# smdesai/mlx-swift-audio

Measured on AMD Instinct MI355X. Metric: audio-sec/s (Whisper large-v3-turbo b=32) at 1/2/4/8 GPU; codec samples/s, higher is better.
Workload: dtype bf16; 1 GPU; Whisper large-v3-turbo bf16, batch=32x30 s synthetic clips per MI355X, log-mel+encode+greedy decode (T=0, timestamps, max_tokens 448, one window per clip), random-init N(0,0.02^2) weights; clips_per_gpu=32, global_batch=32, parallelism=dp1, replicas=3, exchange=none, schedule=pipelined

## Files before the change

include/mia.h:

```cpp
#ifndef MIA_H
#define MIA_H

#include <stddef.h>
#include <stdint.h>

#ifdef __cplusplus
extern "C" {
#endif

typedef struct mia_ctx mia_ctx;
typedef struct mia_whisper mia_whisper;
typedef struct mia_codec mia_codec;
typedef struct mia_lm mia_lm;
typedef struct mia_s3tok mia_s3tok;

typedef enum {
  MIA_OK = 0,
  MIA_ERR_INVALID_ARGUMENT = -1,
  MIA_ERR_MODEL_NOT_LOADED = -2,
  MIA_ERR_INVALID_AUDIO = -3,
  MIA_ERR_OUT_OF_MEMORY = -4,
  MIA_ERR_DEVICE = -5,
  MIA_ERR_UNSUPPORTED = -6
} mia_status;
// ... 18 lines not shown
                       int64_t pad_right, int64_t n_frames_out, void* mel, int out_dtype, int mem);

int mia_logmel_s3(mia_ctx* ctx, const float* pcm, const int64_t* offs, int B, int n_mels,
                  int64_t pad_right, int64_t n_frames_out, void* mel, int out_dtype, int mem);

int64_t mia_mel_s3gen_frames(int64_t n_samples);
int mia_mel_s3gen(mia_ctx* ctx, const float* pcm, int64_t n_samples, float* mel, int mem);

int64_t mia_resample_linear_len(int64_t n_samples, float scale);
int mia_resample_linear(mia_ctx* ctx, const float* x, int64_t n_samples, float scale, float* out, int mem);
int64_t mia_resample_sinc_len(int64_t n_samples, int from_rate, int to_rate);
int mia_resample_sinc_table(int from_rate, int to_rate, float* table, int capacity, int* L_out, int* taps_out);
int mia_resample_sinc(mia_ctx* ctx, const float* x, int64_t n_samples, int from_rate, int to_rate, float* out, int64_t out_capacity,
                      int64_t* n_out, int mem);

int mia_dp_shard_range(int n_items, int rank, int world, int* lo, int* hi);
int mia_dp_shard_cap(int n_items, int world);
int mia_dp_unpack_host(const int32_t* gathered, int n_items, int world, int L, int32_t* dense);
int mia_dp_available(void);
int mia_dp_unique_id(mia_ctx* ctx, void* id128);
int mia_dp_init(mia_ctx* ctx, int rank, int world, const void* unique_id);
int mia_dp_shutdown(mia_ctx* ctx);
int mia_dp_gather_tokens(mia_ctx* ctx, const int32_t* local_tokens, const int32_t* local_counts, int b_local, int L, int n_items,
                         int32_t* all_tokens, int32_t* all_counts);

int mia_op_linear(mia_ctx* ctx, const void* x, int64_t lda, const void* w, const float* bias, const float* r, int64_t ldr,
                  void* y, int64_t ldy, int M, int N, int K, int act, int dtype, int out_f32, int variant, int mem);

int mia_op_linear_epi(mia_ctx* ctx, const void* x, int64_t lda, const void* w, const float* bias, void* y, int64_t ldy, void* vt, int M, int N,
                      int K, int epi, int T, int H, int Tpad, int batch, int dtype, int out_f32, int variant, int mem);

int mia_op_attention_h64(mia_ctx* ctx, const void* qk, int64_t ld_qk, const void* vt, void* out, int64_t ld_out, int B, int T, int H, int Tpad,
                         int dtype, int mem);

int mia_op_conv1d_f32(mia_ctx* ctx, const float* x, int64_t ldx, int T_in, const float* w, const float* bias, const float* r, float* y,
                      int64_t ldy, int T_out, int N, int Cin, int taps, int stride, int dil, int pad, int act);

int mia_dequant_affine(mia_ctx* ctx, const uint32_t* wq, const void* scales, const void* biases, int64_t rows, int64_t cols,
                       int group_size, int bits, int scale_dtype, void* out, int out_dtype, int mem);

int mia_op_attention_f32(mia_ctx* ctx, const float* q, int64_t ldq, const float* k, int64_t ldk, const float* v, int64_t ldv, float* out,
                         int64_t ldo, int B, int T, int H, float scale);

typedef struct {
  const float* X; int64_t ldx; int32_t T_in;
  const float* W; int64_t ldw; int64_t w_phase_stride;
  const float* bias;
  const float* alpha; const float* ralpha;
  float lrelu_slope;
  float* Y; int64_t ldy; int32_t T_out;
  int32_t y_row_mul, y_row_off, y_phase_step;
  const float* R; const float* R2; int64_t ldr;
  const float* noise;
  float out_scale;
  int32_t M, N, Cin, taps, dil, pad;
  int32_t x_row_mul;
  int32_t act;
  int32_t tanh_out;
  const int32_t* phase_len; int32_t x_phase_step;
  int32_t n_seq; int64_t x_seq_step, y_seq_step;
  const int32_t* seq_len; const int32_t* noise_seq_off;
} mia_conv_gemm_desc;
int mia_op_conv_gemm_f32(mia_ctx* ctx, const mia_conv_gemm_desc* d, int phases);

int mia_op_attention_f32_ex(mia_ctx* ctx, const float* q, int64_t ldq, const float* k, int64_t ldk, const float* v, int64_t ldv, const float* p,
                            int64_t ldp, const float* bias_u, const float* bias_v, float* out, int64_t ldo, int B, int T, int H, float scale,
// ... 256 lines not shown
```

mlx-swift-audio_amd/csrc/attention.hip:

```cpp
#include <type_traits>

#include "mia_device.h"
#include "ops.h"

namespace {

constexpr int KV_TILE = 64;
constexpr int TILE_BYTES = 64 * 128;

__device__ __forceinline__ int swap23(int r) {
  return (r & ~12) | ((r & 4) << 1) | ((r & 8) >> 1);
}

template <typename T>
__global__ __launch_bounds__(256, 2) void enc_attention_kernel(const uint16_t* __restrict__ qk, int64_t ld_qk,
                                                               const uint16_t* __restrict__ vt, uint16_t* __restrict__ out,
                                                               int64_t ld_out, int T_len, int Tpad, int H, float scale_log2) {
  __shared__ __attribute__((aligned(16))) char lds[4 * TILE_BYTES];
  const int tid = threadIdx.x, lane = tid & 63, wave = tid >> 6;
  const int nqb = (T_len + 127) / 128;
  int lin = blockIdx.x;
  {
    const int nwg = gridDim.x, q = nwg / 8, r = nwg % 8, xcd = lin % 8;
    lin = (xcd < r ? xcd * (q + 1) : r * (q + 1) + (xcd - r) * q) + lin / 8;
  }
  const int qb = lin % nqb, hb = lin / nqb;
  const int h = hb % H, b = hb / H;
  const int D = H * 64;
  const int q0 = qb * 128 + wave * 32;
  const int lq = lane & 31, lh = lane >> 5;

  s16x8 qf[4];
  {
    int q = q0 + lq; q = q < T_len ? q : T_len - 1;
    const uint16_t* qp = qk + ((int64_t)b * T_len + q) * ld_qk + h * 64 + 8 * lh;
#pragma unroll
    for (int ks = 0; ks < 4; ++ks) qf[ks] = *reinterpret_cast<const s16x8*>(qp + 16 * ks);
  }

  const int s_row = tid >> 3, s_chk = tid & 7;
  const uint16_t* kbase = qk + (int64_t)b * T_len * ld_qk + D + h * 64 + s_chk * 8;
  const uint16_t* vbase = vt + ((int64_t)b * H + h) * 64 * Tpad + s_chk * 8;
  int s_dst[2];
#pragma unroll
  for (int i = 0; i < 2; ++i) {
    const int row = s_row + 32 * i;
    s_dst[i] = row * 128 + ((s_chk ^ ((row >> 1) & 7)) << 4);
  }
  u32x4 rk[2], rv[2];
  auto load_regs = [&](int key0) {
#pragma unroll
    for (int i = 0; i < 2; ++i) {
      const int row = s_row + 32 * i;
      int key = key0 + row; key = key < T_len ? key : T_len - 1;
      rk[i] = *reinterpret_cast<const u32x4*>(kbase + (int64_t)key * ld_qk);
      rv[i] = *reinterpret_cast<const u32x4*>(vbase + (int64_t)row * Tpad + key0);
    }
  };
  auto write_lds = [&](int buf) {
    char* base = lds + buf * 2 * TILE_BYTES;
#pragma unroll
    for (int i = 0; i < 2; ++i) {
      *reinterpret_cast<u32x4*>(base + s_dst[i]) = rk[i];
      *reinterpret_cast<u32x4*>(base + TILE_BYTES + s_dst[i]) = rv[i];
    }
  };

  f32x16 acc_o[2];
#pragma unroll
  for (int i = 0; i < 2; ++i)
#pragma unroll
    for (int r = 0; r < 16; ++r) acc_o[i][r] = 0.f;
  float m_run = -INFINITY, l_run = 0.f;

  const int krow = swap23(lq);
  const int ntiles = (T_len + KV_TILE - 1) / KV_TILE;
  auto tile = [&](int kt, int cur, auto tail_tag) {
    constexpr bool TAIL = decltype(tail_tag)::value;
    const int key0 = kt * KV_TILE;
    if (kt + 1 < ntiles) load_regs(key0 + KV_TILE);
    const char* sk = lds + cur * 2 * TILE_BYTES;
    const char* sv = sk + TILE_BYTES;

    f32x16 acc_s[2];
#pragma unroll
    for (int kb = 0; kb < 2; ++kb) {
#pragma unroll
      for (int r = 0; r < 16; ++r) acc_s[kb][r] = 0.f;
      const int row = kb * 32 + krow;
#pragma unroll
      for (int ks = 0; ks < 4; ++ks) {
        const s16x8 kf = *reinterpret_cast<const s16x8*>(sk + row * 128 + (((2 * ks + lh) ^ ((row >> 1) & 7)) << 4));
        acc_s[kb] = T::mfma32(kf, qf[ks], acc_s[kb]);
      }
    }
    float mloc = -INFINITY;
#pragma unroll
    for (int kb = 0; kb < 2; ++kb)
#pragma unroll
      for (int r = 0; r < 16; ++r) {
        if (TAIL) {
          const int i = (r & 3) + 8 * (r >> 2) + 4 * lh;
          if (key0 + kb * 32 + swap23(i) >= T_len) acc_s[kb][r] = -INFINITY;
        }
        mloc = fmaxf(mloc, acc_s[kb][r]);
      }
    mloc = fmaxf(mloc, __shfl_xor(mloc, 32, 64));
    constexpr float LAZY_LOG2 = 8.0f;
    const bool grow = (mloc - m_run) * scale_log2 > LAZY_LOG2;
    if (__builtin_amdgcn_ballot_w64(grow) != 0ull) {
      const float m_new = grow ? mloc : m_run;
      const float alpha = __builtin_amdgcn_exp2f((m_run - m_new) * scale_log2);
      m_run = m_new;
      l_run *= alpha;
#pragma unroll
      for (int db = 0; db < 2; ++db)
#pragma unroll
        for (int r = 0; r < 16; ++r) acc_o[db][r] *= alpha;
    }
    const float neg_mc = -m_run * scale_log2;
    float lsum = 0.f;
    s16x8 pf[2][2];
#pragma unroll
    for (int kb = 0; kb < 2; ++kb) {
      float p[16];
#pragma unroll
      for (int r = 0; r < 16; ++r) {
        p[r] = __builtin_amdgcn_exp2f(fmaf(acc_s[kb][r], scale_log2, neg_mc));
        lsum += p[r];
      }
#pragma unroll
      for (int s = 0; s < 2; ++s) {
        u32x4 w;
#pragma unroll
        for (int j = 0; j < 4; ++j) w[j] = pack2<T>(p[8 * s + 2 * j], p[8 * s + 2 * j + 1]);
        pf[kb][s] = __builtin_bit_cast(s16x8, w);
      }
    }
    l_run += lsum;

#pragma unroll
    for (int db = 0; db < 2; ++db) {
      const int row = db * 32 + lq;
#pragma unroll
      for (int kb = 0; kb < 2; ++kb)
#pragma unroll
        for (int s = 0; s < 2; ++s) {
          const int chk = kb * 4 + 2 * s + lh;
          const s16x8 vf = *reinterpret_cast<const s16x8*>(sv + row * 128 + ((chk ^ ((row >> 1) & 7)) << 4));
          acc_o[db] = T::mfma32(vf, pf[kb][s], acc_o[db]);
        }
    }
    if (kt + 1 < ntiles) write_lds(cur ^ 1);
    __syncthreads();
  };
  load_regs(0);
  write_lds(0);
  __syncthreads();
  const int nfull = T_len / KV_TILE;
  int cur = 0;
  for (int kt = 0; kt < nfull; ++kt) { tile(kt, cur, std::false_type{}); cur ^= 1; }
  if (nfull < ntiles) tile(nfull, cur, std::true_type{});

  l_run += __shfl_xor(l_run, 32, 64);
  const float inv = 1.0f / l_run;
  const int q = q0 + lq;
  if (q < T_len) {
    uint16_t* op = out + ((int64_t)b * T_len + q) * ld_out + h * 64 + 4 * lh;
#pragma unroll
    for (int db = 0; db < 2; ++db)
#pragma unroll
      for (int g = 0; g < 4; ++g) {
        const float o0 = acc_o[db][4 * g + 0] * inv, o1 = acc_o[db][4 * g + 1] * inv;
        const float o2 = acc_o[db][4 * g + 2] * inv, o3 = acc_o[db][4 * g + 3] * inv;
        *reinterpret_cast<u32x2*>(op + db * 32 + 8 * g) = (u32x2){pack2<T>(o0, o1), pack2<T>(o2, o3)};
      }
  }
}

}

const char* mia_enc_attention_check(int B, int T, int H, int Tpad, int64_t ld_qk, int64_t ld_out) {
  if (B <= 0 || T <= 0 || H <= 0) return "attention: B, T, H must be > 0";
  if (Tpad % 64 || Tpad < T) return "attention: Tpad must be a multiple of 64 and >= T";
  if (ld_qk % 8 || ld_out % 4) return "attention: row strides must keep 16-byte (qk) / 8-byte (out) alignment";
  return nullptr;
}

int mia_enc_attention_launch(const void* qk, int64_t ld_qk, const void* vt, void* out, int64_t ld_out, int B, int T, int H,
                             int Tpad, int dtype, hipStream_t s) {
  dim3 grid(((T + 127) / 128) * H * B), block(256);
  const float scale_log2 = 0.125f * 1.4426950408889634f;
  if (dtype == MIA_F16)
    hipLaunchKernelGGL((enc_attention_kernel<F16>), grid, block, 0, s, (const uint16_t*)qk, ld_qk, (const uint16_t*)vt,
                       (uint16_t*)out, ld_out, T, Tpad, H, scale_log2);
  else
    hipLaunchKernelGGL((enc_attention_kernel<BF16>), grid, block, 0, s, (const uint16_t*)qk, ld_qk, (const uint16_t*)vt,
                       (uint16_t*)out, ld_out, T, Tpad, H, scale_log2);
  return hipGetLastError() == hipSuccess ? 0 : -1;
}
```

mlx-swift-audio_amd/csrc/ops.h:

```cpp
#pragma once
#include <hip/hip_runtime.h>
#include <stdint.h>

#include "../../include/mia.h"

const char* mia_norm_check(int M, int D, int64_t ldx, int64_t ldy);
int mia_norm_launch(const float* x, int64_t ldx, const float* gamma, const float* beta, void* y, int64_t ldy, int M, int D,
                    float eps, bool rms, int out_dtype, hipStream_t s);

const char* mia_enc_attention_check(int B, int T, int H, int Tpad, int64_t ld_qk, int64_t ld_out);
int mia_enc_attention_launch(const void* qk, int64_t ld_qk, const void* vt, void* out, int64_t ld_out, int B, int T, int H,
                             int Tpad, int dtype, hipStream_t s);

struct AttnF32Args {
  const float* q = nullptr; int64_t ldq = 0;
  const float* k = nullptr; int64_t ldk = 0;
  const float* v = nullptr; int64_t ldv = 0;
  const float* p = nullptr; int64_t ldp = 0;
  const float* bias_u = nullptr; const float* bias_v = nullptr;
  float* out = nullptr; int64_t ldo = 0;
  int B = 1, T = 0, H = 0;
  float scale = 0.125f;
  const int32_t* seq_len = nullptr;
  int chunk = 0;
};
const char* mia_attn_f32_check(const AttnF32Args& a);
int mia_attn_f32_launch(const AttnF32Args& a, hipStream_t s);

struct Attn128Args {
  const void* q = nullptr; int64_t ldq = 0;
  const void* k = nullptr; int64_t ldk = 0;
  const void* v = nullptr; int64_t ldv = 0;
  void* out = nullptr; int64_t ldo = 0;
  int B = 1, T = 0, H = 0;
  float scale = 0.08838834764831845f;
  const int32_t* seq_len = nullptr;
  int dtype = MIA_BF16;
};
const char* mia_attn128_check(const Attn128Args& a);
int mia_attn128_launch(const Attn128Args& a, hipStream_t s);

struct FsmnArgs {
  float* x = nullptr; int64_t ldx = 0;
  const void* v = nullptr; int64_t ldv = 0;
  const float* w = nullptr;
// ... 7 lines not shown
```

mlx-swift-audio_amd/csrc/ops_abi.hip:

```cpp
#include "gemm.h"
#include "mia_internal.h"
#include "ops.h"

extern "C" int mia_op_linear(mia_ctx* ctx, const void* x, int64_t lda, const void* w, const float* bias, const float* r, int64_t ldr,
                             void* y, int64_t ldy, int M, int N, int K, int act, int dtype, int out_f32, int variant, int mem) {
  if (!ctx) return MIA_ERR_INVALID_ARGUMENT;
  MIA_CHECK_ARG(ctx, x && w && y, "op_linear: null pointer");
  MIA_CHECK_ARG(ctx, dtype == MIA_BF16 || dtype == MIA_F16, "op_linear: dtype must be MIA_BF16 or MIA_F16");
  MIA_CHECK_ARG(ctx, mem == MIA_MEM_HOST || mem == MIA_MEM_DEVICE, "op_linear: bad mem");
  MIA_CHECK_ARG(ctx, M > 0 && N > 0 && K > 0 && lda >= K && ldy >= N && (!r || ldr >= N), "op_linear: bad shape");
  MIA_HIP(ctx, hipSetDevice(ctx->device));
  GemmArgs g;
  g.M = M; g.N = N; g.K = K; g.lda = lda; g.ldc = ldy; g.ldr = ldr; g.act = act; g.out_f32 = out_f32 ? 1 : 0; g.variant = variant;
  const size_t xb = (size_t)M * lda * 2, wb = (size_t)N * K * 2, yb = (size_t)M * ldy * (out_f32 ? 4 : 2);
  const size_t bb = bias ? (size_t)N * 4 : 0, rb = r ? (size_t)M * ldr * 4 : 0;
  if (mem == MIA_MEM_DEVICE) {
    g.A = x; g.W = w; g.C = y; g.bias = bias; g.R = r;
  } else {
    const size_t o_w = align_up(xb, 256), o_y = o_w + align_up(wb, 256), o_b = o_y + align_up(yb, 256), o_r = o_b + align_up(bb, 256);
    char* ws = (char*)mia_workspace(ctx, o_r + align_up(rb, 256));
    if (!ws) return MIA_ERR_OUT_OF_MEMORY;
    MIA_HIP(ctx, hipMemcpyAsync(ws, x, xb, hipMemcpyHostToDevice, ctx->stream));
    MIA_HIP(ctx, hipMemcpyAsync(ws + o_w, w, wb, hipMemcpyHostToDevice, ctx->stream));
    if (bias) MIA_HIP(ctx, hipMemcpyAsync(ws + o_b, bias, bb, hipMemcpyHostToDevice, ctx->stream));
// ... 29 lines not shown
  }
  MIA_HIP(ctx, hipSetDevice(ctx->device));
  GemmArgs g;
  g.M = M; g.N = N; g.K = K; g.lda = lda; g.ldc = ldy; g.out_f32 = out_f32 ? 1 : 0; g.variant = variant; g.batch = batch;
  g.epi = epi; g.T = T; g.H = H; g.Tpad = Tpad;
  const size_t xb = (size_t)M * lda * 2, wb = (size_t)N * K * 2, bb = bias ? (size_t)N * 4 : 0;
  const size_t yb = epi == MIA_EPI_QKV_VT ? (size_t)(((int64_t)M - 1) * ldy + D2) * 2 : (size_t)B * H * T * 64 * 2;
  const size_t vb = epi == MIA_EPI_QKV_VT ? (size_t)B * H * 64 * Tpad * 2 : 0;
  if (mem == MIA_MEM_DEVICE) {
    g.A = x; g.W = w; g.C = y; g.C2 = vt; g.bias = bias;
  } else {
    const size_t o_w = align_up(xb, 256), o_y = o_w + align_up(wb, 256), o_v = o_y + align_up(yb, 256), o_b = o_v + align_up(vb, 256);
    char* ws = (char*)mia_workspace(ctx, o_b + align_up(bb, 256));
    if (!ws) return MIA_ERR_OUT_OF_MEMORY;
    g.A = ws; g.W = ws + o_w; g.C = ws + o_y; g.C2 = vb ? ws + o_v : nullptr; g.bias = bias ? (const float*)(ws + o_b) : nullptr;
  }
  if (const char* e = mia_gemm_check(g)) return mia_fail(ctx, MIA_ERR_INVALID_ARGUMENT, "%s", e);
  if (mem == MIA_MEM_HOST) {
    MIA_HIP(ctx, hipMemcpyAsync((void*)g.A, x, xb, hipMemcpyHostToDevice, ctx->stream));
    MIA_HIP(ctx, hipMemcpyAsync((void*)g.W, w, wb, hipMemcpyHostToDevice, ctx->stream));
    if (bias) MIA_HIP(ctx, hipMemcpyAsync((void*)g.bias, bias, bb, hipMemcpyHostToDevice, ctx->stream));
    MIA_HIP(ctx, hipMemcpyAsync(g.C, y, yb, hipMemcpyHostToDevice, ctx->stream));
    if (vb) MIA_HIP(ctx, hipMemcpyAsync(g.C2, vt, vb, hipMemcpyHostToDevice, ctx->stream));
  }
  if (mia_gemm_launch(g, dtype, ctx->stream) != 0) return mia_fail(ctx, MIA_ERR_DEVICE, "op_linear_epi: launch failed");
  if (mem == MIA_MEM_HOST) {
    MIA_HIP(ctx, hipMemcpyAsync(y, g.C, yb, hipMemcpyDeviceToHost, ctx->stream));
    if (vb) MIA_HIP(ctx, hipMemcpyAsync(vt, g.C2, vb, hipMemcpyDeviceToHost, ctx->stream));
    MIA_HIP(ctx, hipStreamSynchronize(ctx->stream));
  }
  return MIA_OK;
}

extern "C" int mia_op_attention_h64(mia_ctx* ctx, const void* qk, int64_t ld_qk, const void* vt, void* out, int64_t ld_out, int B, int T, int H,
                                    int Tpad, int dtype, int mem) {
  if (!ctx) return MIA_ERR_INVALID_ARGUMENT;
  MIA_CHECK_ARG(ctx, mem == MIA_MEM_HOST || mem == MIA_MEM_DEVICE, "op_attention_h64: bad mem");
  MIA_CHECK_ARG(ctx, qk && vt && out, "op_attention_h64: null pointer");
  MIA_CHECK_ARG(ctx, dtype == MIA_BF16 || dtype == MIA_F16, "op_attention_h64: dtype must be MIA_BF16 or MIA_F16");
  if (const char* e = mia_enc_attention_check(B, T, H, Tpad, ld_qk, ld_out)) return mia_fail(ctx, MIA_ERR_INVALID_ARGUMENT, "%s", e);
  const int64_t rows = (int64_t)B * T, D = (int64_t)H * 64;
  MIA_CHECK_ARG(ctx, rows < (1ll << 31) && (int64_t)B * H * ((T + 127) / 128) < (1ll << 31), "op_attention_h64: B * T must stay below 2^31");
  MIA_CHECK_ARG(ctx, ld_qk >= 2 * D && ld_out >= D, "op_attention_h64: row strides must cover the row (ld_qk >= 2 * H * 64, ld_out >= H * 64)");
  MIA_CHECK_ARG(ctx, mem == MIA_MEM_HOST || ((((uintptr_t)qk | (uintptr_t)vt) & 15) == 0 && ((uintptr_t)out & 7) == 0),
                "op_attention_h64: qk and vt must be 16-byte aligned, out 8-byte aligned");
  MIA_HIP(ctx, hipSetDevice(ctx->device));
  const void* d_qk = qk; const void* d_vt = vt; void* d_out = out;
  size_t ob = 0;
  if (mem == MIA_MEM_HOST) {
    const size_t qb = (size_t)((rows - 1) * ld_qk + 2 * D) * 2, vb = (size_t)B * H * 64 * Tpad * 2;
    ob = (size_t)((rows - 1) * ld_out + D) * 2;
    const size_t o_v = align_up(qb, 256), o_o = o_v + align_up(vb, 256);
    char* ws = (char*)mia_workspace(ctx, o_o + align_up(ob, 256));
    if (!ws) return MIA_ERR_OUT_OF_MEMORY;
    MIA_HIP(ctx, hipMemcpyAsync(ws + o_o, out, ob, hipMemcpyHostToDevice, ctx->stream));
    MIA_HIP(ctx, hipMemcpyAsync(ws, qk, qb, hipMemcpyHostToDevice, ctx->stream));
    MIA_HIP(ctx, hipMemcpyAsync(ws + o_v, vt, vb, hipMemcpyHostToDevice, ctx->stream));
    d_qk = ws; d_vt = ws + o_v; d_out = ws + o_o;
  }
  if (mia_enc_attention_launch(d_qk, ld_qk, d_vt, d_out, ld_out, B, T, H, Tpad, dtype, ctx->stream))
    return mia_fail(ctx, MIA_ERR_DEVICE, "op_attention_h64: launch failed");
  if (mem == MIA_MEM_HOST) {
    MIA_HIP(ctx, hipMemcpyAsync(out, d_out, ob, hipMemcpyDeviceToHost, ctx->stream));
    MIA_HIP(ctx, hipStreamSynchronize(ctx->stream));
  }
  return MIA_OK;
}

#include "codec.h"
static const char* conv_gemm_abi_check(const ConvGemmArgs& g, int phases) {
  if (!g.X || !g.W || !g.Y) return "null pointer";
  if (phases <= 0 || g.T_in <= 0 || g.T_out <= 0 || g.dil <= 0 || g.x_row_mul <= 0) return "bad argument";
  if (g.ldx < g.Cin || g.ldy < g.N || ((g.R || g.R2) && g.ldr < g.N)) return "row strides must cover the row";
  if (g.gelu < 0 || g.gelu > 6) return "unknown activation";
  return nullptr;
}

extern "C" int mia_op_conv1d_f32(mia_ctx* ctx, const float* x, int64_t ldx, int T_in, const float* w, const float* bias, const float* r, float* y,
                                 int64_t ldy, int T_out, int N, int Cin, int taps, int stride, int dil, int pad, int act) {
  if (!ctx) return MIA_ERR_INVALID_ARGUMENT;
  MIA_CHECK_ARG(ctx, x && w && y && T_in > 0 && T_out > 0 && N > 0 && taps > 0 && stride > 0 && dil > 0, "op_conv1d_f32: bad argument");
  MIA_HIP(ctx, hipSetDevice(ctx->device));
  ConvGemmArgs g;
  g.X = x; g.ldx = ldx; g.T_in = T_in; g.W = w; g.bias = bias; g.Y = y; g.ldy = ldy; g.T_out = T_out; g.R = r; g.ldr = ldy;
  g.M = T_out; g.N = N; g.Cin = Cin; g.taps = taps; g.dil = dil; g.pad = pad; g.x_row_mul = stride; g.gelu = act;
  if (const char* e = conv_gemm_abi_check(g, 1)) return mia_fail(ctx, MIA_ERR_INVALID_ARGUMENT, "op_conv1d_f32: %s", e);
  if (const char* e = codec_conv_gemm_check(g)) return mia_fail(ctx, MIA_ERR_INVALID_ARGUMENT, "%s", e);
  if (codec_conv_gemm_launch(g, 1, ctx->stream)) return mia_fail(ctx, MIA_ERR_DEVICE, "op_conv1d_f32: launch failed");
  return MIA_OK;
}

extern "C" int mia_op_conv_gemm_f32(mia_ctx* ctx, const mia_conv_gemm_desc* d, int phases) {
  if (!ctx) return MIA_ERR_INVALID_ARGUMENT;
  MIA_CHECK_ARG(ctx, d, "op_conv_gemm_f32: null descriptor");
  MIA_HIP(ctx, hipSetDevice(ctx->device));
  ConvGemmArgs g;
  g.X = d->X; g.ldx = d->ldx; g.T_in = d->T_in; g.W = d->W; g.ldw = d->ldw; g.w_phase_stride = d->w_phase_stride; g.bias = d->bias;
  g.alpha = d->alpha; g.ralpha = d->ralpha; g.lrelu_slope = d->lrelu_slope; g.Y = d->Y; g.ldy = d->ldy; g.T_out = d->T_out;
  g.y_row_mul = d->y_row_mul; g.y_row_off = d->y_row_off; g.y_phase_step = d->y_phase_step; g.R = d->R; g.R2 = d->R2; g.ldr = d->ldr;
// ... 264 lines not shown
```

mlx-swift-audio_amd/ops.py:

```python
from __future__ import annotations

import ctypes as C

import numpy as np

from . import _lib
from . import audio as _audio


def _declare(lib):
    if getattr(lib, "_ops_declared", False):
        return
    vp, i32, i64 = C.c_void_p, C.c_int, C.c_int64
    lib.mia_op_linear.restype = i32
    lib.mia_op_linear.argtypes = [vp, vp, i64, vp, vp, vp, i64, vp, i64, i32, i32, i32, i32, i32, i32, i32, i32]
    lib.mia_op_attention_h128.restype = i32
    lib.mia_op_attention_h128.argtypes = [vp, vp, i64, vp, i64, vp, i64, vp, i64, i32, i32, i32, C.c_float, vp, i32, i32]
    lib.mia_op_fsmn_add.restype = i32
    lib.mia_op_fsmn_add.argtypes = [vp, vp, i64, vp, i64, vp, i32, i32, i32, i32, i32, vp, i32, i32]
    lib._ops_declared = True


def to16(a: np.ndarray, dtype: int) -> np.ndarray:
    return np.ascontiguousarray(a, np.float32).astype(np.float16) if dtype == _lib.F16 else _audio.f32_to_bf16(a)
# ... 14 lines not shown
    y = np.empty((M, N), np.float32 if out_f32 else (np.float16 if dtype == _lib.F16 else np.uint16))
    ctx.check(ctx.lib.mia_op_linear(ctx.h, x16.ctypes.data, K, w16.ctypes.data, None if b is None else b.ctypes.data,
                                    None if r is None else r.ctypes.data, N, y.ctypes.data, N, M, N, K,
                                    {None: 0, "gelu": 1, "relu": 2}[act], dtype, 1 if out_f32 else 0, variant, _lib.MEM_HOST))
    return y if out_f32 else from16(y, dtype)


def attention_h128(ctx: _lib.Context, qkv: np.ndarray, B: int, T: int, H: int, scale: float | None = None, seq_len=None,
                   dtype: int = _lib.BF16, fill: float = 0.0) -> np.ndarray:
    _declare(ctx.lib)
    D = H * 128
    assert qkv.shape == (B * T, 3 * D)
    x16 = to16(qkv, dtype)
    out = to16(np.full((B * T, D), fill, np.float32), dtype)
    sl = None if seq_len is None else np.ascontiguousarray(seq_len, np.int32)
    base, es = x16.ctypes.data, x16.itemsize
    ctx.check(ctx.lib.mia_op_attention_h128(ctx.h, base, 3 * D, base + D * es, 3 * D, base + 2 * D * es, 3 * D, out.ctypes.data, D, B, T, H,
                                            float(128 ** -0.5 if scale is None else scale), None if sl is None else sl.ctypes.data,
                                            dtype, _lib.MEM_HOST))
    return from16(out, dtype)


EPI_QKV_VT, EPI_HEADMAJOR = 1, 2


def _declare_enc(lib):
    if getattr(lib, "_enc_ops_declared", False):
        return
    vp, i32, i64 = C.c_void_p, C.c_int, C.c_int64
    lib.mia_op_linear_epi.restype = i32
    lib.mia_op_linear_epi.argtypes = [vp, vp, i64, vp, vp, vp, i64, vp] + [i32] * 12
    lib.mia_op_attention_h64.restype = i32
    lib.mia_op_attention_h64.argtypes = [vp, vp, i64, vp, vp, i64] + [i32] * 6
    lib._enc_ops_declared = True


def bits16(a: np.ndarray, dtype: int) -> np.ndarray:
    return to16(a, dtype).view(np.uint16)


def from_bits16(a: np.ndarray, dtype: int) -> np.ndarray:
    return from16(a.view(np.float16) if dtype == _lib.F16 else a, dtype)


def enc_attention_buffers(q: np.ndarray, k: np.ndarray, v: np.ndarray, B: int, T: int, H: int, Tpad: int, ld_qk: int, pad_fill: float, dtype: int):
    D = H * 64
    assert q.shape == k.shape == v.shape == (B * T, D)
    qk = bits16(np.full((B * T, ld_qk), pad_fill, np.float32), dtype)
    qk[:, :D], qk[:, D:2 * D] = bits16(q, dtype), bits16(k, dtype)
    vt = bits16(np.full((B, H, 64, Tpad), pad_fill, np.float32), dtype)
    vt[..., T:min(Tpad, (T + 63) // 64 * 64)] = 0
    vt[..., :T] = bits16(v, dtype).reshape(B, T, H, 64).transpose(0, 2, 3, 1)
    return qk, vt


def attention_h64(ctx: _lib.Context, q: np.ndarray, k: np.ndarray, v: np.ndarray, B: int, T: int, H: int, *, Tpad: int | None = None,
                  ld_qk: int | None = None, ld_out: int | None = None, fill: float = 0.0, pad_fill: float = 0.0,
                  dtype: int = _lib.BF16) -> np.ndarray:
    _declare_enc(ctx.lib)
    D = H * 64
    Tpad = (T + 63) // 64 * 64 if Tpad is None else Tpad
    ld_qk = 2 * D if ld_qk is None else ld_qk
    ld_out = D if ld_out is None else ld_out
    qk, vt = enc_attention_buffers(q, k, v, B, T, H, Tpad, ld_qk, pad_fill, dtype)
    out = bits16(np.full((B * T, ld_out), fill, np.float32), dtype)
    ctx.check(ctx.lib.mia_op_attention_h64(ctx.h, qk.ctypes.data, ld_qk, vt.ctypes.data, out.ctypes.data, ld_out, B, T, H, Tpad, dtype, _lib.MEM_HOST))
    return from_bits16(out, dtype)


def attention_h64_device(ctx: _lib.Context, qk, vt, out, B: int, T: int, H: int, Tpad: int, ld_qk: int, ld_out: int, dtype: int) -> None:
    _declare_enc(ctx.lib)
    assert qk.is_cuda and vt.is_cuda and out.is_cuda
    _run(ctx, lambda: ctx.lib.mia_op_attention_h64(ctx.h, _ptr(qk), ld_qk, _ptr(vt), _ptr(out), ld_out, B, T, H, Tpad, dtype, _lib.MEM_DEVICE))


def linear_epi(ctx: _lib.Context, x: np.ndarray, w: np.ndarray, bias, y: np.ndarray, vt, *, epi: int, T: int, H: int, Tpad: int = 0,
               ldy: int | None = None, dtype: int = _lib.BF16, variant: int = 3, out_f32: bool = False, batch: int = 1, N: int | None = None):
    _declare_enc(ctx.lib)
    M, K = x.shape
    x16, w16 = to16(x, dtype), to16(w, dtype)
    b = None if bias is None else np.ascontiguousarray(bias, np.float32)
    yo = np.array(y, np.uint16, order="C")
    vo = None if vt is None else np.array(vt, np.uint16, order="C")
    ldy = int(ldy if ldy is not None else (yo.shape[1] if yo.ndim == 2 else H * 64))
    ctx.check(ctx.lib.mia_op_linear_epi(ctx.h, x16.ctypes.data, K, w16.ctypes.data, None if b is None else b.ctypes.data, yo.ctypes.data, ldy,
                                        None if vo is None else vo.ctypes.data, M, int(w.shape[0] if N is None else N), K, int(epi), int(T), int(H),
                                        int(Tpad), int(batch), dtype, 1 if out_f32 else 0, int(variant), _lib.MEM_HOST))
    return yo, vo, from_bits16(yo, dtype), None if vo is None else from_bits16(vo, dtype)


def linear_epi_device(ctx: _lib.Context, x, w, bias, y, vt, *, M: int, N: int, K: int, epi: int, T: int, H: int, Tpad: int, ldy: int,
                      dtype: int, variant: int = 3) -> None:
    _declare_enc(ctx.lib)
    _run(ctx, lambda: ctx.lib.mia_op_linear_epi(ctx.h, _ptr(x), K, _ptr(w), _ptr(bias), _ptr(y), ldy, _ptr(vt), M, N, K, int(epi), T, H, Tpad, 1,
                                                dtype, 0, int(variant), _lib.MEM_DEVICE))


def fsmn_add(ctx: _lib.Context, x: np.ndarray, v: np.ndarray, w: np.ndarray, left: int, B: int = 1, seq_len=None,
             dtype: int = _lib.BF16) -> np.ndarray:
    _declare(ctx.lib)
    rows, D = x.shape
    T = rows // B
    xo = np.array(x, np.float32, order="C")
    v16 = to16(v, dtype)
    w32 = np.ascontiguousarray(w, np.float32)
    sl = None if seq_len is None else np.ascontiguousarray(seq_len, np.int32)
# ... 190 lines not shown
```

Measured before the change: 4734 audio-sec/s.

## Add direct-to-LDS triple-buffered encoder attention with 64-query-per-wave variant

Rewrites the encoder flash-attention kernel so K/V tiles are loaded with global_load_lds DMA into a three-slot LDS ring instead of staging through registers and a double buffer. This is meant to remove register staging and a sync per tile. It also adds a variant where each wave handles two 32-query blocks, interleaving their QK, softmax and PV MFMAs so one K/V tile is reused across more queries. A heuristic picks the 256-query variant for long sequences with enough workgroups and the DMA 128-query kernel otherwise. The cost is higher register pressure and fewer workgroups, plus a more complex wait and barrier scheme.

```diff
diff --git a/include/mia.h b/include/mia.h
--- a/include/mia.h
+++ b/include/mia.h
@@ -74,6 +74,8 @@
 
 int mia_op_attention_h64(mia_ctx* ctx, const void* qk, int64_t ld_qk, const void* vt, void* out, int64_t ld_out, int B, int T, int H, int Tpad,
                          int dtype, int mem);
+int mia_op_attention_h64_variant(mia_ctx* ctx, const void* qk, int64_t ld_qk, const void* vt, void* out, int64_t ld_out, int B, int T, int H,
+                                 int Tpad, int dtype, int variant, int mem);
 
 int mia_op_conv1d_f32(mia_ctx* ctx, const float* x, int64_t ldx, int T_in, const float* w, const float* bias, const float* r, float* y,
                       int64_t ldy, int T_out, int N, int Cin, int taps, int stride, int dil, int pad, int act);
diff --git a/mlx-swift-audio_amd/csrc/attention.hip b/mlx-swift-audio_amd/csrc/attention.hip
--- a/mlx-swift-audio_amd/csrc/attention.hip
+++ b/mlx-swift-audio_amd/csrc/attention.hip
@@ -12,13 +12,27 @@
   return (r & ~12) | ((r & 4) << 1) | ((r & 8) >> 1);
 }
 
-template <typename T>
-__global__ __launch_bounds__(256, 2) void enc_attention_kernel(const uint16_t* __restrict__ qk, int64_t ld_qk,
-                                                               const uint16_t* __restrict__ vt, uint16_t* __restrict__ out,
-                                                               int64_t ld_out, int T_len, int Tpad, int H, float scale_log2) {
-  __shared__ __attribute__((aligned(16))) char lds[4 * TILE_BYTES];
+__device__ __forceinline__ void glds16(const void* g, void* l) {
+  __builtin_amdgcn_global_load_lds((const __attribute__((address_space(1))) void*)g,
+                                   (__attribute__((address_space(3))) void*)l, 16, 0, 0);
+}
+
+#define ATT_BAR()                                 \
+  do {                                            \
+    asm volatile("" ::: "memory");                \
+    __builtin_amdgcn_s_barrier();                 \
+    asm volatile("" ::: "memory");                \
+  } while (0)
+
+constexpr int SLOT_BYTES = 2 * TILE_BYTES;
+
+template <typename T, int NQ, bool DMA>
+__device__ __forceinline__ void enc_attention_body(char* lds, const uint16_t* __restrict__ qk, int64_t ld_qk,
+                                                   const uint16_t* __restrict__ vt, uint16_t* __restrict__ out, int64_t ld_out,
+                                                   int T_len, int Tpad, int H, float scale_log2) {
   const int tid = threadIdx.x, lane = tid & 63, wave = tid >> 6;
-  const int nqb = (T_len + 127) / 128;
+  constexpr int QWG = 128 * NQ;
+  const int nqb = (T_len + QWG - 1) / QWG;
   int lin = blockIdx.x;
   {
     const int nwg = gridDim.x, q = nwg / 8, r = nwg % 8, xcd = lin % 8;
@@ -27,25 +41,33 @@
   const int qb = lin % nqb, hb = lin / nqb;
   const int h = hb % H, b = hb / H;
   const int D = H * 64;
-  const int q0 = qb * 128 + wave * 32;
+  const int q0 = qb * QWG + wave * (32 * NQ);
   const int lq = lane & 31, lh = lane >> 5;
 
-  s16x8 qf[4];
-  {
-    int q = q0 + lq; q = q < T_len ? q : T_len - 1;
-    const uint16_t* qp = qk + ((int64_t)b * T_len + q) * ld_qk + h * 64 + 8 * lh;
-#pragma unroll
-    for (int ks = 0; ks < 4; ++ks) qf[ks] = *reinterpret_cast<const s16x8*>(qp + 16 * ks);
-  }
-
-  const int s_row = tid >> 3, s_chk = tid & 7;
+  s16x8 qf[NQ][4];
+  auto load_q = [&]() {
+#pragma unroll
+    for (int n = 0; n < NQ; ++n) {
+      int q = q0 + 32 * n + lq; q = q < T_len ? q : T_len - 1;
+      const uint16_t* qp = qk + ((int64_t)b * T_len + q) * ld_qk + h * 64 + 8 * lh;
+#pragma unroll
+      for (int ks = 0; ks < 4; ++ks) qf[n][ks] = *reinterpret_cast<const s16x8*>(qp + 16 * ks);
+    }
+  };
+  if (!DMA) load_q();
+
+  const int s_row = tid >> 3, s_pos = tid & 7;
+  const int s_chk = DMA ? (s_pos ^ ((s_row >> 1) & 7)) : s_pos;
   const uint16_t* kbase = qk + (int64_t)b * T_len * ld_qk + D + h * 64 + s_chk * 8;
   const uint16_t* vbase = vt + ((int64_t)b * H + h) * 64 * Tpad + s_chk * 8;
+  const int ntiles = (T_len + KV_TILE - 1) / KV_TILE;
+  const int nfull = T_len / KV_TILE;
+
   int s_dst[2];
 #pragma unroll
   for (int i = 0; i < 2; ++i) {
     const int row = s_row + 32 * i;
-    s_dst[i] = row * 128 + ((s_chk ^ ((row >> 1) & 7)) << 4);
+    s_dst[i] = row * 128 + ((s_pos ^ ((row >> 1) & 7)) << 4);
   }
   u32x4 rk[2], rv[2];
   auto load_regs = [&](int key0) {
@@ -58,7 +80,7 @@
     }
   };
   auto write_lds = [&](int buf) {
-    char* base = lds + buf * 2 * TILE_BYTES;
+    char* base = lds + buf * SLOT_BYTES;
 #pragma unroll
     for (int i = 0; i < 2; ++i) {
       *reinterpret_cast<u32x4*>(base + s_dst[i]) = rk[i];
@@ -66,116 +88,239 @@
     }
   };
 
-  f32x16 acc_o[2];
-#pragma unroll
-  for (int i = 0; i < 2; ++i)
-#pragma unroll
-    for (int r = 0; r < 16; ++r) acc_o[i][r] = 0.f;
-  float m_run = -INFINITY, l_run = 0.f;
+  const uint16_t* kp[2];
+  const uint16_t* vp[2];
+#pragma unroll
+  for (int i = 0; i < 2; ++i) {
+    kp[i] = kbase + (int64_t)(s_row + 32 * i) * ld_qk;
+    vp[i] = vbase + (int64_t)(s_row + 32 * i) * Tpad;
+  }
+  const int64_t k_step = (int64_t)KV_TILE * ld_qk;
+  int slot_issue = 0;
+  char* const lds_wave = lds + __builtin_amdgcn_readfirstlane(wave) * 1024;
+  auto issue_full = [&]() {
+    char* dst = lds_wave + slot_issue * SLOT_BYTES;
+#pragma unroll
+    for (int i = 0; i < 2; ++i) {
+      glds16(kp[i], dst + i * 4096);
+      glds16(vp[i], dst + TILE_BYTES + i * 4096);
+      kp[i] += k_step;
+      vp[i] += KV_TILE;
+    }
+    slot_issue = slot_issue == 2 ? 0 : slot_issue + 1;
+  };
+  auto issue = [&](int kt) {
+    if (kt < nfull) {
+      issue_full();
+    } else {
+      char* dst = lds_wave + slot_issue * SLOT_BYTES;
+#pragma unroll
+      for (int i = 0; i < 2; ++i) {
+        int key = kt * KV_TILE + s_row + 32 * i; key = key < T_len ? key : T_len - 1;
+        glds16(kbase + (int64_t)key * ld_qk, dst + i * 4096);
+        glds16(vp[i], dst + TILE_BYTES + i * 4096);
+      }
+      slot_issue = slot_issue == 2 ? 0 : slot_issue + 1;
+    }
+  };
+
+  f32x16 acc_o[NQ][2];
+  float m_run[NQ], l_run[NQ];
+#pragma unroll
+  for (int n = 0; n < NQ; ++n) {
+#pragma unroll
+    for (int i = 0; i < 2; ++i)
+#pragma unroll
+      for (int r = 0; r < 16; ++r) acc_o[n][i][r] = 0.f;
+    m_run[n] = -INFINITY; l_run[n] = 0.f;
+  }
 
   const int krow = swap23(lq);
-  const int ntiles = (T_len + KV_TILE - 1) / KV_TILE;
-  auto tile = [&](int kt, int cur, auto tail_tag) {
+  auto tile = [&](int kt, int cur, auto tail_tag, auto steady_tag) {
     constexpr bool TAIL = decltype(tail_tag)::value;
+    constexpr bool STEADY = decltype(steady_tag)::value;
     const int key0 = kt * KV_TILE;
-    if (kt + 1 < ntiles) load_regs(key0 + KV_TILE);
-    const char* sk = lds + cur * 2 * TILE_BYTES;
+    if (DMA) {
+      if (STEADY || kt + 1 < ntiles) asm volatile("s_waitcnt vmcnt(4) lgkmcnt(0)" ::: "memory");
+      else asm volatile("s_waitcnt vmcnt(0) lgkmcnt(0)" ::: "memory");
+      ATT_BAR();
+      if (STEADY) issue_full();
+      else if (kt + 2 < ntiles) issue(kt + 2);
+    } else {
+      if (kt + 1 < ntiles) load_regs(key0 + KV_TILE);
+    }
+    const char* sk = lds + cur * SLOT_BYTES;
     const char* sv = sk + TILE_BYTES;
 
-    f32x16 acc_s[2];
-#pragma unroll
-    for (int kb = 0; kb < 2; ++kb) {
-#pragma unroll
-      for (int r = 0; r < 16; ++r) acc_s[kb][r] = 0.f;
-      const int row = kb * 32 + krow;
-#pragma unroll
-      for (int ks = 0; ks < 4; ++ks) {
-        const s16x8 kf = *reinterpret_cast<const s16x8*>(sk + row * 128 + (((2 * ks + lh) ^ ((row >> 1) & 7)) << 4));
-        acc_s[kb] = T::mfma32(kf, qf[ks], acc_s[kb]);
-      }
-    }
-    float mloc = -INFINITY;
-#pragma unroll
-    for (int kb = 0; kb < 2; ++kb)
-#pragma unroll
-      for (int r = 0; r < 16; ++r) {
-        if (TAIL) {
-          const int i = (r & 3) + 8 * (r >> 2) + 4 * lh;
-          if (key0 + kb * 32 + swap23(i) >= T_len) acc_s[kb][r] = -INFINITY;
-        }
-        mloc = fmaxf(mloc, acc_s[kb][r]);
-      }
-    mloc = fmaxf(mloc, __shfl_xor(mloc, 32, 64));
-    constexpr float LAZY_LOG2 = 8.0f;
-    const bool grow = (mloc - m_run) * scale_log2 > LAZY_LOG2;
-    if (__builtin_amdgcn_ballot_w64(grow) != 0ull) {
-      const float m_new = grow ? mloc : m_run;
-      const float alpha = __builtin_amdgcn_exp2f((m_run - m_new) * scale_log2);
-      m_run = m_new;
-      l_run *= alpha;
+    f32x16 acc_s[NQ][2];
+    s16x8 kf[2][4], vf[2][4], pf[NQ][2][2];
+    auto read_k = [&]() {
+#pragma unroll
+      for (int kb = 0; kb < 2; ++kb) {
+        const int row = kb * 32 + krow;
+#pragma unroll
+        for (int ks = 0; ks < 4; ++ks)
+          kf[kb][ks] = *reinterpret_cast<const s16x8*>(sk + row * 128 + (((2 * ks + lh) ^ ((row >> 1) & 7)) << 4));
+      }
+    };
+    auto read_v = [&]() {
+#pragma unroll
+      for (int db = 0; db < 2; ++db) {
+        const int row = db * 32 + lq;
+#pragma unroll
+        for (int c = 0; c < 4; ++c) {
+          const int chk = 2 * c + lh;
+          vf[db][c] = *reinterpret_cast<const s16x8*>(sv + row * 128 + ((chk ^ ((row >> 1) & 7)) << 4));
+        }
+      }
+    };
+    auto s_mma = [&](int n, int kb) {
+#pragma unroll
+      for (int r = 0; r < 16; ++r) acc_s[n][kb][r] = 0.f;
+#pragma unroll
+      for (int ks = 0; ks < 4; ++ks) acc_s[n][kb] = T::mfma32(kf[kb][ks], qf[n][ks], acc_s[n][kb]);
+    };
+    auto soft_max = [&](int n) {
+      float mloc = -INFINITY;
+      int left = T_len - key0;
+      if (TAIL && NQ > 1) asm volatile("" : "+v"(left));
+#pragma unroll
+      for (int kb = 0; kb < 2; ++kb)
+#pragma unroll
+        for (int r = 0; r < 16; ++r) {
+          if (TAIL) {
+            const int i = (r & 3) + 8 * (r >> 2) + 4 * lh;
+            if (kb * 32 + swap23(i) >= left) acc_s[n][kb][r] = -INFINITY;
+          }
+          mloc = fmaxf(mloc, acc_s[n][kb][r]);
+        }
+      return fmaxf(mloc, __shfl_xor(mloc, 32, 64));
+    };
+    auto rescale = [&](int n, float mloc) {
+      constexpr float LAZY_LOG2 = 8.0f;
+      const bool grow = (mloc - m_run[n]) * scale_log2 > LAZY_LOG2;
+      if (__builtin_amdgcn_ballot_w64(grow) != 0ull) {
+        const float m_new = grow ? mloc : m_run[n];
+        const float alpha = __builtin_amdgcn_exp2f((m_run[n] - m_new) * scale_log2);
+        m_run[n] = m_new;
+        l_run[n] *= alpha;
+#pragma unroll
+        for (int db = 0; db < 2; ++db)
+#pragma unroll
+          for (int r = 0; r < 16; ++r) acc_o[n][db][r] *= alpha;
+      }
+    };
+    auto soft_exp = [&](int n) {
+      const float neg_mc = -m_run[n] * scale_log2;
+      float lsum = 0.f;
+#pragma unroll
+      for (int kb = 0; kb < 2; ++kb) {
+        float p[16];
+#pragma unroll
+        for (int r = 0; r < 16; ++r) {
+          p[r] = __builtin_amdgcn_exp2f(fmaf(acc_s[n][kb][r], scale_log2, neg_mc));
+          lsum += p[r];
+        }
+#pragma unroll
+        for (int s = 0; s < 2; ++s) {
+          u32x4 w;
+#pragma unroll
+          for (int j = 0; j < 4; ++j) w[j] = pack2<T>(p[8 * s + 2 * j], p[8 * s + 2 * j + 1]);
+          pf[n][kb][s] = __builtin_bit_cast(s16x8, w);
+        }
+      }
+      l_run[n] += lsum;
+    };
+    auto pv_mma = [&](int n, int db) {
+#pragma unroll
+      for (int kb = 0; kb < 2; ++kb)
+#pragma unroll
+        for (int s = 0; s < 2; ++s) acc_o[n][db] = T::mfma32(vf[db][kb * 2 + s], pf[n][kb][s], acc_o[n][db]);
+    };
+
+    read_k();
+    if (NQ == 1) {
+      s_mma(0, 0); s_mma(0, 1);
+      rescale(0, soft_max(0));
+      soft_exp(0);
+      read_v();
+      pv_mma(0, 0); pv_mma(0, 1);
+    } else {
+      constexpr int N1 = NQ - 1;
+      s_mma(0, 0); s_mma(0, 1);
+      s_mma(N1, 0);
+      const float m0 = soft_max(0);
+      rescale(0, m0);
+      s_mma(N1, 1);
+      soft_exp(0);
+      read_v();
+      pv_mma(0, 0);
+      const float m1 = soft_max(N1);
+      rescale(N1, m1);
+      pv_mma(0, 1);
+      soft_exp(N1);
+      pv_mma(N1, 0); pv_mma(N1, 1);
+    }
+    if (!DMA) {
+      if (kt + 1 < ntiles) write_lds(cur ^ 1);
+      __syncthreads();
+    }
+  };
+  if (DMA) {
+    issue(0);
+    if (ntiles > 1) issue(1);
+    load_q();
+#pragma unroll
+    for (int n = 0; n < NQ; ++n)
+#pragma unroll
+      for (int ks = 0; ks < 4; ++ks) asm volatile("" : "+v"(qf[n][ks]));
+    int cur = 0, kt = 0;
+    for (; kt + 2 < nfull; ++kt) { tile(kt, cur, std::false_type{}, std::true_type{}); cur = cur == 2 ? 0 : cur + 1; }
+    for (; kt < nfull; ++kt) { tile(kt, cur, std::false_type{}, std::false_type{}); cur = cur == 2 ? 0 : cur + 1; }
+    if (nfull < ntiles) tile(nfull, cur, std::true_type{}, std::false_type{});
+  } else {
+    load_regs(0);
+    write_lds(0);
+    __syncthreads();
+    int cur = 0;
+    for (int kt = 0; kt < nfull; ++kt) { tile(kt, cur, std::false_type{}, std::false_type{}); cur ^= 1; }
+    if (nfull < ntiles) tile(nfull, cur, std::true_type{}, std::false_type{});
+  }
+
+#pragma unroll
+  for (int n = 0; n < NQ; ++n) {
+    l_run[n] += __shfl_xor(l_run[n], 32, 64);
+    const float inv = 1.0f / l_run[n];
+    int q = q0 + 32 * n + lq;
+    if (NQ > 1) asm volatile("" : "+v"(q));
+    if (q < T_len) {
+      uint16_t* op = out + ((int64_t)b * T_len + q) * ld_out + h * 64 + 4 * lh;
 #pragma unroll
       for (int db = 0; db < 2; ++db)
 #pragma unroll
-        for (int r = 0; r < 16; ++r) acc_o[db][r] *= alpha;
-    }
-    const float neg_mc = -m_run * scale_log2;
-    float lsum = 0.f;
-    s16x8 pf[2][2];
-#pragma unroll
-    for (int kb = 0; kb < 2; ++kb) {
-      float p[16];
-#pragma unroll
-      for (int r = 0; r < 16; ++r) {
-        p[r] = __builtin_amdgcn_exp2f(fmaf(acc_s[kb][r], scale_log2, neg_mc));
-        lsum += p[r];
-      }
-#pragma unroll
-      for (int s = 0; s < 2; ++s) {
-        u32x4 w;
-#pragma unroll
-        for (int j = 0; j < 4; ++j) w[j] = pack2<T>(p[8 * s + 2 * j], p[8 * s + 2 * j + 1]);
-        pf[kb][s] = __builtin_bit_cast(s16x8, w);
-      }
-    }
-    l_run += lsum;
-
-#pragma unroll
-    for (int db = 0; db < 2; ++db) {
-      const int row = db * 32 + lq;
-#pragma unroll
-      for (int kb = 0; kb < 2; ++kb)
-#pragma unroll
-        for (int s = 0; s < 2; ++s) {
-          const int chk = kb * 4 + 2 * s + lh;
-          const s16x8 vf = *reinterpret_cast<const s16x8*>(sv + row * 128 + ((chk ^ ((row >> 1) & 7)) << 4));
-          acc_o[db] = T::mfma32(vf, pf[kb][s], acc_o[db]);
-        }
-    }
-    if (kt + 1 < ntiles) write_lds(cur ^ 1);
-    __syncthreads();
-  };
-  load_regs(0);
-  write_lds(0);
-  __syncthreads();
-  const int nfull = T_len / KV_TILE;
-  int cur = 0;
-  for (int kt = 0; kt < nfull; ++kt) { tile(kt, cur, std::false_type{}); cur ^= 1; }
-  if (nfull < ntiles) tile(nfull, cur, std::true_type{});
-
-  l_run += __shfl_xor(l_run, 32, 64);
-  const float inv = 1.0f / l_run;
-  const int q = q0 + lq;
-  if (q < T_len) {
-    uint16_t* op = out + ((int64_t)b * T_len + q) * ld_out + h * 64 + 4 * lh;
-#pragma unroll
-    for (int db = 0; db < 2; ++db)
-#pragma unroll
-      for (int g = 0; g < 4; ++g) {
-        const float o0 = acc_o[db][4 * g + 0] * inv, o1 = acc_o[db][4 * g + 1] * inv;
-        const float o2 = acc_o[db][4 * g + 2] * inv, o3 = acc_o[db][4 * g + 3] * inv;
-        *reinterpret_cast<u32x2*>(op + db * 32 + 8 * g) = (u32x2){pack2<T>(o0, o1), pack2<T>(o2, o3)};
-      }
-  }
+        for (int g = 0; g < 4; ++g) {
+          const float o0 = acc_o[n][db][4 * g + 0] * inv, o1 = acc_o[n][db][4 * g + 1] * inv;
+          const float o2 = acc_o[n][db][4 * g + 2] * inv, o3 = acc_o[n][db][4 * g + 3] * inv;
+          *reinterpret_cast<u32x2*>(op + db * 32 + 8 * g) = (u32x2){pack2<T>(o0, o1), pack2<T>(o2, o3)};
+        }
+    }
+  }
+}
+
+template <typename T, bool DMA>
+__global__ __launch_bounds__(256, 2) void enc_attention_kernel(const uint16_t* __restrict__ qk, int64_t ld_qk,
+                                                               const uint16_t* __restrict__ vt, uint16_t* __restrict__ out,
+                                                               int64_t ld_out, int T_len, int Tpad, int H, float scale_log2) {
+  __shared__ __attribute__((aligned(16))) char lds[(DMA ? 3 : 2) * SLOT_BYTES];
+  enc_attention_body<T, 1, DMA>(lds, qk, ld_qk, vt, out, ld_out, T_len, Tpad, H, scale_log2);
+}
+
+template <typename T>
+__global__ __launch_bounds__(256, 2) void enc_attn_q64_kernel(const uint16_t* __restrict__ qk, int64_t ld_qk,
+                                                              const uint16_t* __restrict__ vt, uint16_t* __restrict__ out,
+                                                              int64_t ld_out, int T_len, int Tpad, int H, float scale_log2) {
+  __shared__ __attribute__((aligned(16))) char lds[3 * SLOT_BYTES];
+  enc_attention_body<T, 2, true>(lds, qk, ld_qk, vt, out, ld_out, T_len, Tpad, H, scale_log2);
 }
 
 }
@@ -187,15 +332,31 @@
   return nullptr;
 }
 
+template <typename E>
+static void launch_variant(int variant, dim3 block, hipStream_t s, const uint16_t* qk, int64_t ld_qk, const uint16_t* vt, uint16_t* out,
+                           int64_t ld_out, int B, int T, int H, int Tpad, float scale_log2) {
+  const dim3 g128(((T + 127) / 128) * H * B), g256(((T + 255) / 256) * H * B);
+  switch (variant) {
+    case MIA_ATT_REG128: hipLaunchKernelGGL((enc_attention_kernel<E, false>), g128, block, 0, s, qk, ld_qk, vt, out, ld_out, T, Tpad, H, scale_log2); break;
+    case MIA_ATT_DMA128: hipLaunchKernelGGL((enc_attention_kernel<E, true>), g128, block, 0, s, qk, ld_qk, vt, out, ld_out, T, Tpad, H, scale_log2); break;
+    default: hipLaunchKernelGGL((enc_attn_q64_kernel<E>), g256, block, 0, s, qk, ld_qk, vt, out, ld_out, T, Tpad, H, scale_log2); break;
+  }
+}
+
+int mia_enc_attention_launch_variant(const void* qk, int64_t ld_qk, const void* vt, void* out, int64_t ld_out, int B, int T, int H,
+                                     int Tpad, int dtype, int variant, hipStream_t s) {
+  if (variant < 0 || variant >= MIA_ATT_NVARIANTS) return -1;
+  const float scale_log2 = 0.125f * 1.4426950408889634f;
+  if (dtype == MIA_F16)
+    launch_variant<F16>(variant, dim3(256), s, (const uint16_t*)qk, ld_qk, (const uint16_t*)vt, (uint16_t*)out, ld_out, B, T, H, Tpad, scale_log2);
+  else
+    launch_variant<BF16>(variant, dim3(256), s, (const uint16_t*)qk, ld_qk, (const uint16_t*)vt, (uint16_t*)out, ld_out, B, T, H, Tpad, scale_log2);
+  return hipGetLastError() == hipSuccess ? 0 : -1;
+}
+
 int mia_enc_attention_launch(const void* qk, int64_t ld_qk, const void* vt, void* out, int64_t ld_out, int B, int T, int H,
                              int Tpad, int dtype, hipStream_t s) {
-  dim3 grid(((T + 127) / 128) * H * B), block(256);
-  const float scale_log2 = 0.125f * 1.4426950408889634f;
-  if (dtype == MIA_F16)
-    hipLaunchKernelGGL((enc_attention_kernel<F16>), grid, block, 0, s, (const uint16_t*)qk, ld_qk, (const uint16_t*)vt,
-                       (uint16_t*)out, ld_out, T, Tpad, H, scale_log2);
-  else
-    hipLaunchKernelGGL((enc_attention_kernel<BF16>), grid, block, 0, s, (const uint16_t*)qk, ld_qk, (const uint16_t*)vt,
-                       (uint16_t*)out, ld_out, T, Tpad, H, scale_log2);
-  return hipGetLastError() == hipSuccess ? 0 : -1;
-}
+  const int64_t nwg256 = (int64_t)((T + 255) / 256) * H * B;
+  const int variant = T >= 1024 && nwg256 >= 480 ? MIA_ATT_DMA256 : MIA_ATT_DMA128;
+  return mia_enc_attention_launch_variant(qk, ld_qk, vt, out, ld_out, B, T, H, Tpad, dtype, variant, s);
+}
diff --git a/mlx-swift-audio_amd/csrc/ops.h b/mlx-swift-audio_amd/csrc/ops.h
--- a/mlx-swift-audio_amd/csrc/ops.h
+++ b/mlx-swift-audio_amd/csrc/ops.h
@@ -11,6 +11,9 @@
 const char* mia_enc_attention_check(int B, int T, int H, int Tpad, int64_t ld_qk, int64_t ld_out);
 int mia_enc_attention_launch(const void* qk, int64_t ld_qk, const void* vt, void* out, int64_t ld_out, int B, int T, int H,
                              int Tpad, int dtype, hipStream_t s);
+enum { MIA_ATT_REG128 = 0, MIA_ATT_DMA128 = 1, MIA_ATT_DMA256 = 2, MIA_ATT_NVARIANTS = 3 };
+int mia_enc_attention_launch_variant(const void* qk, int64_t ld_qk, const void* vt, void* out, int64_t ld_out, int B, int T, int H,
+                                     int Tpad, int dtype, int variant, hipStream_t s);
 
 struct AttnF32Args {
   const float* q = nullptr; int64_t ldq = 0;
diff --git a/mlx-swift-audio_amd/csrc/ops_abi.hip b/mlx-swift-audio_amd/csrc/ops_abi.hip
--- a/mlx-swift-audio_amd/csrc/ops_abi.hip
+++ b/mlx-swift-audio_amd/csrc/ops_abi.hip
@@ -85,9 +85,10 @@
   return MIA_OK;
 }
 
-extern "C" int mia_op_attention_h64(mia_ctx* ctx, const void* qk, int64_t ld_qk, const void* vt, void* out, int64_t ld_out, int B, int T, int H,
-                                    int Tpad, int dtype, int mem) {
-  if (!ctx) return MIA_ERR_INVALID_ARGUMENT;
+static int op_attention_h64(mia_ctx* ctx, const void* qk, int64_t ld_qk, const void* vt, void* out, int64_t ld_out, int B, int T, int H,
+                            int Tpad, int dtype, int variant, int mem) {
+  if (!ctx) return MIA_ERR_INVALID_ARGUMENT;
+  MIA_CHECK_ARG(ctx, variant >= -1 && variant < MIA_ATT_NVARIANTS, "op_attention_h64: unknown kernel variant");
   MIA_CHECK_ARG(ctx, mem == MIA_MEM_HOST || mem == MIA_MEM_DEVICE, "op_attention_h64: bad mem");
   MIA_CHECK_ARG(ctx, qk && vt && out, "op_attention_h64: null pointer");
   MIA_CHECK_ARG(ctx, dtype == MIA_BF16 || dtype == MIA_F16, "op_attention_h64: dtype must be MIA_BF16 or MIA_F16");
@@ -111,13 +112,22 @@
     MIA_HIP(ctx, hipMemcpyAsync(ws + o_v, vt, vb, hipMemcpyHostToDevice, ctx->stream));
     d_qk = ws; d_vt = ws + o_v; d_out = ws + o_o;
   }
-  if (mia_enc_attention_launch(d_qk, ld_qk, d_vt, d_out, ld_out, B, T, H, Tpad, dtype, ctx->stream))
+  if (variant < 0 ? mia_enc_attention_launch(d_qk, ld_qk, d_vt, d_out, ld_out, B, T, H, Tpad, dtype, ctx->stream)
+                  : mia_enc_attention_launch_variant(d_qk, ld_qk, d_vt, d_out, ld_out, B, T, H, Tpad, dtype, variant, ctx->stream))
     return mia_fail(ctx, MIA_ERR_DEVICE, "op_attention_h64: launch failed");
   if (mem == MIA_MEM_HOST) {
     MIA_HIP(ctx, hipMemcpyAsync(out, d_out, ob, hipMemcpyDeviceToHost, ctx->stream));
     MIA_HIP(ctx, hipStreamSynchronize(ctx->stream));
   }
   return MIA_OK;
+}
+extern "C" int mia_op_attention_h64(mia_ctx* ctx, const void* qk, int64_t ld_qk, const void* vt, void* out, int64_t ld_out, int B, int T, int H,
+                                    int Tpad, int dtype, int mem) {
+  return op_attention_h64(ctx, qk, ld_qk, vt, out, ld_out, B, T, H, Tpad, dtype, -1, mem);
+}
+extern "C" int mia_op_attention_h64_variant(mia_ctx* ctx, const void* qk, int64_t ld_qk, const void* vt, void* out, int64_t ld_out, int B, int T,
+                                            int H, int Tpad, int dtype, int variant, int mem) {
+  return op_attention_h64(ctx, qk, ld_qk, vt, out, ld_out, B, T, H, Tpad, dtype, variant, mem);
 }
 
 #include "codec.h"
diff --git a/mlx-swift-audio_amd/ops.py b/mlx-swift-audio_amd/ops.py
--- a/mlx-swift-audio_amd/ops.py
+++ b/mlx-swift-audio_amd/ops.py
@@ -70,6 +70,8 @@
     lib.mia_op_linear_epi.argtypes = [vp, vp, i64, vp, vp, vp, i64, vp] + [i32] * 12
     lib.mia_op_attention_h64.restype = i32
     lib.mia_op_attention_h64.argtypes = [vp, vp, i64, vp, vp, i64] + [i32] * 6
+    lib.mia_op_attention_h64_variant.restype = i32
+    lib.mia_op_attention_h64_variant.argtypes = [vp, vp, i64, vp, vp, i64] + [i32] * 7
     lib._enc_ops_declared = True
 
 
@@ -106,10 +108,37 @@
     return from_bits16(out, dtype)
 
 
+ATT_REG128, ATT_DMA128, ATT_DMA256 = 0, 1, 2
+ATT_VARIANTS = {"reg128": ATT_REG128, "dma128": ATT_DMA128, "dma256": ATT_DMA256}
+
+
+def attention_h64_bits(ctx: _lib.Context, q: np.ndarray, k: np.ndarray, v: np.ndarray, B: int, T: int, H: int, *, variant: int = -1,
+                       Tpad: int | None = None, ld_qk: int | None = None, ld_out: int | None = None, fill: float = 0.0,
+                       pad_fill: float = 0.0, dtype: int = _lib.BF16) -> np.ndarray:
+    _declare_enc(ctx.lib)
+    D = H * 64
+    Tpad = (T + 63) // 64 * 64 if Tpad is None else Tpad
+    ld_qk = 2 * D if ld_qk is None else ld_qk
+    ld_out = D if ld_out is None else ld_out
+    qk, vt = enc_attention_buffers(q, k, v, B, T, H, Tpad, ld_qk, pad_fill, dtype)
+    out = bits16(np.full((B * T, ld_out), fill, np.float32), dtype)
+    ctx.check(ctx.lib.mia_op_attention_h64_variant(ctx.h, qk.ctypes.data, ld_qk, vt.ctypes.data, out.ctypes.data, ld_out, B, T, H, Tpad, dtype,
+                                                   variant, _lib.MEM_HOST))
+    return out
+
+
 def attention_h64_device(ctx: _lib.Context, qk, vt, out, B: int, T: int, H: int, Tpad: int, ld_qk: int, ld_out: int, dtype: int) -> None:
     _declare_enc(ctx.lib)
     assert qk.is_cuda and vt.is_cuda and out.is_cuda
     _run(ctx, lambda: ctx.lib.mia_op_attention_h64(ctx.h, _ptr(qk), ld_qk, _ptr(vt), _ptr(out), ld_out, B, T, H, Tpad, dtype, _lib.MEM_DEVICE))
+
+
+def attention_h64_device_variant(ctx: _lib.Context, qk, vt, out, B: int, T: int, H: int, Tpad: int, ld_qk: int, ld_out: int, dtype: int,
+                                 variant: int) -> None:
+    _declare_enc(ctx.lib)
+    assert qk.is_cuda and vt.is_cuda and out.is_cuda
+    _run(ctx, lambda: ctx.lib.mia_op_attention_h64_variant(ctx.h, _ptr(qk), ld_qk, _ptr(vt), _ptr(out), ld_out, B, T, H, Tpad, dtype, variant,
+                                                           _lib.MEM_DEVICE))
 
 
 def linear_epi(ctx: _lib.Context, x: np.ndarray, w: np.ndarray, bias, y: np.ndarray, vt, *, epi: int, T: int, H: int, Tpad: int = 0,
```

After: 4796 audio-sec/s, median of 6. +1.3%, better.
